# szemenyeim/DynEnv

Hardware: AMD Instinct MI355X
Metric: agent-steps/s (higher is better)
Workload: dtype f64

## Files before the change

dynenv_amd/csrc/driving_kernels.hip:

```cpp
#include "driving_dev.h"

__constant__ DrvConst C;

#include "driving_host.h"

struct DrvMailbox {
  double p1x[DRV_NS][2], p1y[DRV_NS][2], p2x[DRV_NS][2], p2y[DRV_NS][2], nx[DRV_NS], ny[DRV_NS];
  int hash[DRV_NS][2], count[DRV_NS], flag[DRV_NS];
};
struct DrvObsStage {
  float carRow[DRV_MAXA][8];
  float goal[DRV_MAXA][2];
  float shared[DRV_MAXO * 4 + DRV_MAXP * 2 + DRV_LANE_ROWS * 5];
};
#ifdef DRV_PROFILE
#define DRV_PROF(...) __VA_ARGS__
#else
#define DRV_PROF(...)
#endif
#define DRV_CLIST 128
struct __align__(16) DrvLds {
  double px[DRV_NB], py[DRV_NB], vx[DRV_NB], vy[DRV_NB], ang[DRV_NB], w[DRV_NB], vbx[DRV_NB], vby[DRV_NB], wb[DRV_NB];
  double minv[DRV_NB], iinv[DRV_NB];
  double rc[16], rs[16], rotAng[16];
// ... 684 lines not shown
  }
  double* const fX = biasLane ? L.vbx : L.vx;
  double* const fY = biasLane ? L.vby : L.vy;
  double* const fW = biasLane ? L.wb : L.w;
  const bool aDyn = bodyA < DRV_SLOT_OBST, bDyn = bodyB < DRV_SLOT_OBST;
  a.v = b.v = v2(0.0, 0.0); a.w = b.w = 0.0;
  const int nSteps = maxLevel + 1 + period * 9;
  int due = myLevel, passes = 0;
  const int ra = body_rd(bodyA), rb = body_rd(bodyB), wa = body_wr(bodyA), wb_ = body_wr(bodyB);
#define DRV_SPLIT_PASS(q)                                                                   \
  {                                                                                         \
    const V2 vr = relative_velocity(a, b, r1[q], r2[q]);                                    \
    const double vn = vdot_f(vr, n);                                                        \
    const double t0 = cq[q] + (biasLane ? -vn : vn);                                        \
    const double old = acc[q];                                                              \
    acc[q] = dms_acc_clamp0(biasLane ? t0 : -t0, nM[q], old);                               \
    const double dj = acc[q] - old;                                                         \
    const V2 jr = vrotate_f(n, v2(dj, 0.0));                                                \
    const V2 jl = vmul(n, dj);                                                              \
    const V2 jj = biasLane ? jl : jr;                                                       \
    apply_impulse(a, vneg(jj), r1[q]);                                                      \
    apply_impulse(b, jj, r2[q]);                                                            \
  }
  for (int t = 0; t < nSteps; ++t) {
    if (active && t == due && passes < 10) {
      a.v = v2(fX[ra], fY[ra]); a.w = fW[ra];
      b.v = v2(fX[rb], fY[rb]); b.w = fW[rb];
      DRV_SPLIT_PASS(0)
      if (count > 1) DRV_SPLIT_PASS(1)
      fX[wa] = a.v.x; fY[wa] = a.v.y; fW[wa] = a.w;
      fX[wb_] = b.v.x; fY[wb_] = b.v.y; fW[wb_] = b.w;
      due += period; ++passes;
    }
    __syncthreads();
  }
#undef DRV_SPLIT_PASS
  DrvSplitRet r;
  r.jt0 = jt0; r.jt1 = jt1; r.pk = pk; r.pair = pair; r.bits = bits3;
  r.jn0 = acc[0]; r.jn1 = acc[1];
  r.jb0 = lane_read_d(acc[0], (lane + 32) & 63); r.jb1 = lane_read_d(acc[1], (lane + 32) & 63);
  return r;
}

DRV_PROF(__device__ unsigned long long g_dbgw[4096 * 12];)
DRV_PROF(__device__ unsigned long long g_dbgp[4096 * 8];)
DRV_PROF(__device__ unsigned long long g_dbgr[16];)
DRV_PROF(__device__ unsigned long long g_dbgl[4096 * 8];)
DRV_PROF(__device__ unsigned long long g_dbgs[4096 * 8];)
DRV_PROF(DE_DEV int prof_any(int v) { const uint64_t m = wave_ballot(v != 0); return m ? bcast_i(v, __builtin_ctzll(m)) : 0; })
#ifndef DRV_CONTACT_INLINE
#define DRV_CONTACT_INLINE __forceinline__
#endif

DE_OOL int drv_prestep_solve(int lane, int nCarPed, int pk, int a_pair, int bodyA, int bodyB, int myLevel,
                                             int maxLevel_, int anyActive_, double jn0, double jn1, double jt0, double jt1) {
  DrvLds& L = g_L;
  DrvMailbox& M = L.u.mb;
  int a_state = pk & 0xFF;
  int a_count = (pk >> 8) & 0xFF, a_age = (pk >> 16) & 0xFF;
  bool touched = (pk >> 24) & 1, freeMe = (pk >> 25) & 1, hashSame = (pk >> 26) & 1, prevInert = (pk >> 27) & 1;
  bool skipped = (pk >> 28) & 1, slotOcc = (pk >> 29) & 1, active = (pk >> 30) & 1;
  const bool isCar = lane < (uniform_i(nCarPed) & 0xFF), isPed = lane >= DRV_SLOT_PED && lane < DRV_SLOT_PED + (uniform_i(nCarPed) >> 8);
  const int maxLevel = (int)(signed char)(uniform_i(maxLevel_) & 0xFF), period = uniform_i(maxLevel_) >> 8;
  const uint64_t activeMask = uniform_i(anyActive_) ? 1ull : 0ull;
DRV_PROF(const unsigned long long P0 = __builtin_amdgcn_s_memtime();)
  double jn[2] = {jn0, jn1}, jt[2] = {jt0, jt1};
  V2 n = v2(0.0, 0.0), r1[2], r2[2];
  r1[0] = r1[1] = r2[0] = r2[1] = v2(0.0, 0.0);
  double nMass[2] = {0.0, 0.0}, tMass[2] = {0.0, 0.0}, bias[2] = {0.0, 0.0}, bounce[2] = {0.0, 0.0}, jBias[2] = {0.0, 0.0};
  const double arb_e = 0.05 * 0.05, arb_u = 0.0 * 0.0;
  bool restIn = false;
  if (active) {
    BodyV a, b;
    body_load(L, bodyA, a);
    body_load(L, bodyB, b);
    restIn = a.v.x == 0.0 && a.v.y == 0.0 && a.w == 0.0 && b.v.x == 0.0 && b.v.y == 0.0 && b.w == 0.0;
    r1[0] = vsub(v2(M.p1x[lane][0], M.p1y[lane][0]), a.p);
    r2[0] = vsub(v2(M.p2x[lane][0], M.p2y[lane][0]), b.p);
    if (a_count > 1) {
      r1[1] = vsub(v2(M.p1x[lane][1], M.p1y[lane][1]), a.p);
      r2[1] = vsub(v2(M.p2x[lane][1], M.p2y[lane][1]), b.p);
    }
    n = v2(M.nx[lane], M.ny[lane]);
    V2 body_delta = vsub(b.p, a.p);
#pragma unroll
    for (int c = 0; c < 2; ++c) {
      if (c == 0 || a_count > 1) {
        nMass[c] = 1.0 / (k_scalar_body(a, r1[c], n) + k_scalar_body(b, r2[c], n));
        double dist = vdot_f(vadd(vsub(r2[c], r1[c]), body_delta), n);
        bias[c] = -DE_CONTACT_BIAS_COEF * fmin_cp(0.0, dist + DE_COLLISION_SLOP) / DE_DT;
        jBias[c] = 0.0;
        bounce[c] = vdot_f(relative_velocity(a, b, r1[c], r2[c]), n) * arb_e;
      }
    }
  }
  __syncthreads();
DRV_PROF(const unsigned long long P1 = __builtin_amdgcn_s_memtime();)

  velocity_update(L, lane, isCar, isPed);
DRV_PROF(int profMode = 0; const unsigned long long P2 = __builtin_amdgcn_s_memtime();)
  bool tookSplit = false;
  if (activeMask && maxLevel == 0) {
    __syncthreads();
    if (active) {
      BodyV a, b;
      body_load(L, bodyA, a);
      body_load(L, bodyB, b);
      if (a_state != ARB_FIRST) arb_warm_start(a, b, n, r1, r2, jn, jt, a_count);
      if (wave_ballot(!arb_is_bias_only(a, b, jn, jt, bounce, a_count)) == 0ull) {
DRV_PROF(profMode = 1;)
#pragma unroll 1
        for (int iter = 0; iter < 10; ++iter)
          if (wave_ballot(arb_apply_bias_only(a, b, n, r1, r2, nMass, bias, jBias, a_count)) == 0ull) break;
      } else {
DRV_PROF(profMode = 2;)
#pragma unroll 1
        for (int iter = 0; iter < 10; ++iter) arb_apply_impulse(a, b, n, r1, r2, nMass, tMass, bias, bounce, jBias, jn, jt, a_count, arb_u);
      }
      body_store_vel(L, bodyA, a);
      body_store_vel(L, bodyB, b);
    }
    __syncthreads();
  } else if (activeMask) {
    __syncthreads();
    for (int lv = 0; lv <= maxLevel; ++lv) {
      if (active && myLevel == lv && a_state != ARB_FIRST) {
        BodyV a, b;
        body_load(L, bodyA, a);
        body_load(L, bodyB, b);
        arb_warm_start(a, b, n, r1, r2, jn, jt, a_count);
        body_store_vel(L, bodyA, a);
        body_store_vel(L, bodyB, b);
      }
      __syncthreads();
    }
    BodyV a, b;
    bool biasOnly = true;
    if (active) {
      body_load(L, bodyA, a); body_load(L, bodyB, b);
      biasOnly = arb_is_bias_only(a, b, jn, jt, bounce, a_count);
    }
    const int nSteps = maxLevel + 1 + period * 9;
    int due = myLevel, passes = 0;
DRV_PROF(profMode = wave_ballot(!biasOnly) == 0ull ? 3 : 4;)
    if (wave_ballot(!biasOnly) == 0ull) {
      const int ra = body_rd(bodyA), rb = body_rd(bodyB), wa = body_wr(bodyA), wb_ = body_wr(bodyB);
      for (int t = 0; t < nSteps; ++t) {
        if (active && t == due && passes < 10) {
          a.vb = v2(L.vbx[ra], L.vby[ra]); a.wb = L.wb[ra];
          b.vb = v2(L.vbx[rb], L.vby[rb]); b.wb = L.wb[rb];
          arb_apply_bias_only(a, b, n, r1, r2, nMass, bias, jBias, a_count);
          L.vbx[wa] = a.vb.x; L.vby[wa] = a.vb.y; L.wb[wa] = a.wb;
          L.vbx[wb_] = b.vb.x; L.vby[wb_] = b.vb.y; L.wb[wb_] = b.wb;
          due += period; ++passes;
        }
        __syncthreads();
      }
    } else [[unlikely]] {
      const int bits3 = (restIn ? 1 : 0) | (bias[0] == 0.0 ? 2 : 0) | (bias[1] == 0.0 ? 4 : 0);
      const DrvSplitRet sr = drv_solve_general_split(lane, myLevel, bodyA | (bodyB << 8), maxLevel_, nMass[0], nMass[1], bias[0], bias[1], bounce[0],
                                                     bounce[1], jn[0], jn[1], jt[0], jt[1], pk, a_pair, bits3);
      lane = fresh_lane();
      pk = sr.pk; a_pair = sr.pair;
      a_state = pk & 0xFF; a_count = (pk >> 8) & 0xFF; a_age = (pk >> 16) & 0xFF;
      touched = (pk >> 24) & 1; freeMe = (pk >> 25) & 1; hashSame = (pk >> 26) & 1; prevInert = (pk >> 27) & 1;
      skipped = (pk >> 28) & 1; slotOcc = (pk >> 29) & 1; active = (pk >> 30) & 1;
      restIn = (sr.bits & 1) != 0;
      bias[0] = (sr.bits & 2) ? 0.0 : 1.0; bias[1] = (sr.bits & 4) ? 0.0 : 1.0;
      jn[0] = sr.jn0; jn[1] = sr.jn1; jBias[0] = sr.jb0; jBias[1] = sr.jb1; jt[0] = sr.jt0; jt[1] = sr.jt1;
      tookSplit = true;
    }
  }
DRV_PROF(const unsigned long long P3 = __builtin_amdgcn_s_memtime();)
  const bool wasNormal = a_state == ARB_NORMAL;
  if (active && a_state == ARB_FIRST) a_state = ARB_NORMAL;
  bool steady = true;
  if (slotOcc && !skipped) {
    steady = touched && !freeMe && hashSame;
    if (steady && a_state != ARB_IGNORE) {
      steady = a_state == ARB_NORMAL && wasNormal && restIn && L.s_jn0[lane] == jn[0] && L.s_jt0[lane] == jt[0] &&
               L.s_jn1[lane] == jn[1] && L.s_jt1[lane] == jt[1];
      if (steady) {
        const int i = a_pair >> 8, j = a_pair & 0xFF;
        steady = L.vx[i] == 0.0 && L.vy[i] == 0.0 && L.w[i] == 0.0;
        if (j < DRV_SLOT_OBST) steady = steady && L.vx[j] == 0.0 && L.vy[j] == 0.0 && L.w[j] == 0.0;
      }
    }
  }
  const bool allSteady = wave_ballot(!steady) == 0ull;
  bool inert = true;
  if (slotOcc && skipped) inert = prevInert;
  else if (slotOcc) {
    inert = touched && !freeMe &&
            (a_state == ARB_IGNORE ||
             (a_state == ARB_NORMAL && wasNormal && bias[0] == 0.0 && bias[1] == 0.0 && jn[0] == 0.0 && jt[0] == 0.0 &&
              jn[1] == 0.0 && jt[1] == 0.0 && jBias[0] == 0.0 && jBias[1] == 0.0));
  }
  if (slotOcc) {
    if (freeMe) L.s_pair[lane] = 0xFFFF;
    L.s_meta[lane] = a_state | (a_count << 8) | (a_age << 16) | (steady ? (1 << 24) : 0) | (inert ? (1 << 25) : 0);
    if (touched) { L.s_jn0[lane] = jn[0]; L.s_jt0[lane] = jt[0]; L.s_jn1[lane] = jn[1]; L.s_jt1[lane] = jt[1]; }
  }
  const bool allInert = wave_ballot(!inert) == 0ull;
DRV_PROF(if (lane == 0 && blockIdx.x < 4096) { unsigned long long* d = g_dbgp + blockIdx.x * 8; const unsigned long long P4 = __builtin_amdgcn_s_memtime(); d[2] += (P1 - P0) + ((P4 - P3) << 32); d[3] += (P2 - P1) + ((P3 - P2) << 32); })
  return (allInert ? 2 : 0) | (allSteady ? 4 : 0) | (tookSplit ? 8 : 0) DRV_PROF(| (prof_any(profMode) << 4));
}
struct ContactRet {
  uint64_t occ;
  int err;
};

__device__ DRV_CONTACT_INLINE ContactRet drv_contact_path(int lane, int cand, int dirty, int light, int A, int nCarPed, uint64_t occ) {
  const bool isCar = lane < A, isPed = lane >= DRV_SLOT_PED && lane < DRV_SLOT_PED + (nCarPed >> 8);
  DrvLds& L = g_L;
  int err = 0;
  asm volatile("" : "+v"(lane));
DRV_PROF(const unsigned long long T0 = __builtin_amdgcn_s_memtime();)
  DrvMailbox& M = L.u.mb;
  if (lane < DRV_NS) M.flag[lane] = 0;
  __syncthreads();
  bool lightOk = false;
  int savedN = uniform_i(L.clistN);
  int spair = lane < DRV_NS ? L.s_pair[lane] : -1;
DRV_PROF(int profCand = 0;)
#pragma unroll 1
  for (int mode = light ? 0 : 1; mode < 2; ++mode) {
  const int bits = mode == 0 ? dirty : cand;
  bool lightBad = false;
  int nCand = 0;
  if (mode == 1 && savedN >= 0) nCand = savedN;
  else {
#pragma unroll
  for (int i = 0; i < DRV_MAXA; ++i) {
    const bool c = (bits >> i) & 1;
    const uint64_t m = wave_ballot(c);
    if (c) {
      const int idx = nCand + (int)__builtin_amdgcn_mbcnt_hi((uint32_t)(m >> 32), __builtin_amdgcn_mbcnt_lo((uint32_t)m, 0u));
      if (idx < DRV_CLIST) L.clist[idx] = (unsigned short)((i << 8) | lane); else err |= 1;
    }
    nCand += __popcll(m);
  }
  savedN = mode == 1 && nCand <= DRV_CLIST ? nCand : -1;
  if (lane == 0) L.clistN = savedN;
  if (nCand > DRV_CLIST) nCand = DRV_CLIST;
  }
DRV_PROF(profCand += nCand;)
  __syncthreads();
DRV_PROF(const unsigned long long N1 = __builtin_amdgcn_s_memtime(); unsigned long long nMath = 0ull;)
  if (mode == 0) {
    bool owns = false;
    for (int k = lane; k < nCand; k += 64) {
      const int pr = (int)L.clist[k];
      for (uint64_t mm = occ; mm; mm &= mm - 1) owns = owns || bcast_i(spair, __builtin_ctzll(mm)) == pr;
    }
    if (wave_ballot(owns) != 0ull) continue;
  }
#pragma unroll 1
  for (int pass = 0; pass * 16 < nCand; ++pass) {
// ... 181 lines not shown
    }
    cleanSlot = cleanSlot && (myBodies & dirtyBodies) == 0;
  }
  const bool skipped = cleanSlot;
  {
    int keep = 0;
    const uint64_t skipLanes = wave_ballot(skipped);
    for (uint64_t mm = skipLanes; mm; mm &= mm - 1) keep |= bcast_i(myBodies, __builtin_ctzll(mm));
    if ((isCar || isPed) && !((keep >> lane) & 1)) { L.vbx[lane] = 0.0; L.vby[lane] = 0.0; L.wb[lane] = 0.0; }
  }

DRV_PROF(const unsigned long long U4 = __builtin_amdgcn_s_memtime();)
  const bool active = solvable && !skipped;
  const uint64_t activeMask = wave_ballot(active);
  int myLevel = 0, maxLevel = -1, period = 1;
  const int nActive = __popcll(activeMask);
  const bool lvHit = uniform_u64(c_active) == activeMask;
  if (!lvHit && lane == 0) L.sActive = activeMask;
  if (nActive == 1) maxLevel = 0;
  else if (nActive > 1 && lvHit) {
    myLevel = c_level;
    maxLevel = (int)(signed char)(uniform_i(c_meta) & 0xFF);
    period = uniform_i(c_meta) >> 8;
  } else if (nActive > 1) {
    if (!haveRank && nTouched > 1)
      for (uint64_t mm = touchedMask; mm; mm &= mm - 1) {
        int b = __builtin_ctzll(mm);
        int pk = bcast_i(a_pair, b);
        rank += (pk < a_pair) ? 1 : 0;
      }
    int bl = 0;
    const int bodyAB = bodyA | (bodyB << 8);
    for (int k = 0; k < nTouched; ++k) {
      uint64_t who = wave_ballot(active && rank == k);
      if (who == 0ull) continue;
      int b = __builtin_ctzll(who);
      const int ab = bcast_i(bodyAB, b), ba = ab & 0xFF, bb2 = ab >> 8;
      const int pa = ba < DRV_SLOT_OBST ? bcast_i(bl, ba) : 0, pb = bb2 < DRV_SLOT_OBST ? bcast_i(bl, bb2) : 0;
      const int la = pa & 0xFF, lb = pb & 0xFF;
      int lv = la > lb ? la : lb;
      const int fa = (pa >> 8) - 1, fb = (pb >> 8) - 1;
      const int lo = fa < 0 ? fb : (fb < 0 ? fa : (fa < fb ? fa : fb));
      if (lo >= 0 && lv - lo + 1 > period) period = lv - lo + 1;
      if (lane == b) myLevel = lv;
      if (lane == ba || lane == bb2) bl = (lv + 1) | (((bl >> 8) ? (bl >> 8) : lv + 1) << 8);
      maxLevel = lv > maxLevel ? lv : maxLevel;
    }
    if (lane < DRV_NS) L.sLevel[lane] = (unsigned char)myLevel;
    if (lane == 0) L.sLvMeta = (maxLevel & 0xFF) | (period << 8);
  }

DRV_PROF(const unsigned long long T2 = __builtin_amdgcn_s_memtime();)
DRV_PROF(if (lane == 0 && blockIdx.x < 4096) { unsigned long long* d = g_dbgs + blockIdx.x * 8; d[0] += U1 - T1; d[1] += U2 - U1; d[2] += U3 - U2; d[3] += U4 - U3; d[4] += T2 - U4; })
  const int solveBits = drv_prestep_solve(lane, nCarPed,
                                          (a_state & 0xFF) | ((a_count & 0xFF) << 8) | ((a_age & 0xFF) << 16) | (touched ? 1 << 24 : 0) | (freeMe ? 1 << 25 : 0) |
                                              (hashSame ? 1 << 26 : 0) | (prevInert ? 1 << 27 : 0) | (skipped ? 1 << 28 : 0) | (slotOcc ? 1 << 29 : 0) | (active ? 1 << 30 : 0),
                                          a_pair, bodyA, bodyB, myLevel, (maxLevel & 0xFF) | (period << 8), activeMask != 0ull ? 1 : 0, jn[0], jn[1], jt[0], jt[1]);
  occ &= ~freeMask;
DRV_PROF(const unsigned long long T3 = T2, T4 = T2, T5 = __builtin_amdgcn_s_memtime(); const int profModeW = (uniform_i(solveBits) >> 4) & 7;)
DRV_PROF(if (lane == 0 && blockIdx.x < 4096) { unsigned long long* d = g_dbgp + blockIdx.x * 8; d[0] += T1 - T0; d[1] += T2 - T1; d[2] += T3 - T2; d[3] += T4 - T3; d[4] += T5 - T4; d[5] += 1ull + (light ? (1ull << 16) : 0ull); d[6] += (unsigned long long)(maxLevel + 1) + ((unsigned long long)(maxLevel + 1) << (12 * profModeW)); d[7] += (unsigned long long)nTouched + ((unsigned long long)profCand << 16); })
  {
    ContactRet ret;
    ret.occ = occ; ret.err = err | (uniform_i(solveBits) & 6) | ((uniform_i(solveBits) & 8) << 1);
    return ret;
  }
}

DE_OOL int drv_partial_obs_fused(PvIn in, uint64_t seed, int A, int* envi, int env_id_offset, int e, int nPedObst, int elapsed,
                                 uint32_t episode, int noiseTypeAgents, double magn, float* __restrict__ obs, int budgetCycles);
#ifndef DRV_DEFER_MIN_CONTACT
#define DRV_DEFER_MIN_CONTACT 5
#endif
#ifndef DRV_PV_DEADLINE_PCT
#define DRV_PV_DEADLINE_PCT 110
#endif
#ifndef DRV_FUSED_AGENTS
#define DRV_FUSED_AGENTS 10
#endif
struct DrvLightRet {
  int cand, dirty, bits;
};
struct DrvSeedOnly { uint64_t seed; };
DE_OOL DrvLightRet drv_light_substep(int it_, int lane, int A_, int nPed_, int nObst_, int elapsed_,
                                                      uint32_t seedLo, uint32_t seedHi, uint32_t genv_, uint32_t episode_, int stateBits) {
  DrvLds& L = g_L;
DRV_PROF(const unsigned long long Q0 = __builtin_amdgcn_s_memtime();)
  const int lastCand = L.lastCand[lane];
  const int it = uniform_i(it_), A = uniform_i(A_), nPed = uniform_i(nPed_), nObst = uniform_i(nObst_), elapsed = uniform_i(elapsed_);
  const uint32_t genv = (uint32_t)uniform_i((int)genv_), episode = (uint32_t)uniform_i((int)episode_);
  DrvSeedOnly S;
  S.seed = ((uint64_t)(uint32_t)uniform_i((int)seedHi) << 32) | (uint64_t)(uint32_t)uniform_i((int)seedLo);
  const bool isCar = lane < A;
  const bool isPed = lane >= DRV_SLOT_PED && lane < DRV_SLOT_PED + nPed;
  const bool isBody = isCar || isPed;
  const bool vbValid = (uniform_i(stateBits) & 1) != 0;
  bool aabbValid = (uniform_i(stateBits) & 2) != 0;
    bool turned = false;
    const int bi = lane & (DRV_NB - 1), ci = lane & 15;
    int f = L.flags[bi];
    double px = L.px[bi], py = L.py[bi], vx = L.vx[bi], vy = L.vy[bi], ang = L.ang[bi];
    const double w = L.w[bi];
    const double vbx = vbValid ? L.vbx[bi] : 0.0, vby = vbValid ? L.vby[bi] : 0.0, wb = vbValid ? L.wb[bi] : 0.0;
    double rcv = L.rc[ci], rsv = L.rs[ci], rotAngv = L.rotAng[ci], cosRel0v = L.cosRel0[ci];
    const double goalx = L.goalx[ci], goaly = L.goaly[ci], dprev = L.dprev[ci], chx = L.chx[ci], chy = L.chy[ci];
    double rew = L.rewAcc[ci], posrew = L.posAcc[ci];
    int moving = L.moving[bi];
    if (!isBody) { f = 0; px = 0.0; py = 0.0; vx = 0.0; vy = 0.0; }
    if (isCar) {
      if (it == 0) {
        const int actPk = (int)L.act[lane];
// ... 271 lines not shown
    const int k = atomicAdd(&S.iso[nxt], 1);
    if (k < DRV_ISO_LIST) S.iso[DRV_ISO_HDR + nxt * DRV_ISO_LIST + k] = e;
  }
  __atomic_store_n(&S.iso_done[e], tick, __ATOMIC_RELAXED);
}

template <bool PARTIAL>
DE_DEV void drv_step_body(const DrvState& S, const int* __restrict__ actions, float* __restrict__ obs, double* __restrict__ rewards,
                          uint8_t* __restrict__ dones, float* __restrict__ pobs, int pvNoise, double pvMagn) {
  const unsigned long long isoT0 = __builtin_amdgcn_s_memtime();
DRV_PROF(const unsigned long long KS = isoT0;)
  DrvLds& L = g_L;
  int lane = threadIdx.x;
  const int tick = drv_launch_tick(S);
  if (!S.tick_src && blockIdx.x == 0 && lane == 0) { S.iso[13] = S.tick; S.iso[14] = S.pv_par; }
  const int e = drv_iso_assign(S, lane, tick);
  if (e < 0) return;
DRV_PROF(if (lane < 8 && e < 4096) { g_dbgp[e * 8 + lane] = 0ull; g_dbgs[e * 8 + lane] = 0ull; })
  const int A = S.A;
  int* envi = S.envi + (size_t)e * EI_COUNT;
  int elapsed = uniform_i(envi[EI_ELAPSED]);
  int allFinished = uniform_i(envi[EI_ALLFIN]);
  const int nPed = uniform_i(envi[EI_NPED]);
  const int nObst = uniform_i(envi[EI_NOBST]);
  const uint32_t episode = (uint32_t)uniform_i(envi[EI_EPISODE]);
  uint64_t occ = (uint64_t)(uint32_t)uniform_i(envi[EI_OCC]);
  if (occ != 0ull) __builtin_amdgcn_s_setprio(3);
  else if (PARTIAL) __builtin_amdgcn_s_setprio(1);
  const uint32_t genv = (uint32_t)(S.env_id_offset + e);

  const bool isCar = lane < A;
  const bool isPed = lane >= DRV_SLOT_PED && lane < DRV_SLOT_PED + nPed;
  const bool isBody = isCar || isPed;
  const int g_act0 = actions[((size_t)e * A + (isCar ? lane : 0)) * 2 + 0], g_act1 = actions[((size_t)e * A + (isCar ? lane : 0)) * 2 + 1];
  const int g_lastCand = S.lastcand[(size_t)e * 64 + lane];
  load_env(S, L, e, lane, A, nPed, nObst, occ);

  {
    int act0 = isCar ? g_act0 : 1, act1 = isCar ? g_act1 : 1;
    const bool bad = (unsigned)act0 > 2u || (unsigned)act1 > 2u;
    if (bad) { act0 = 1; act1 = 1; }
    if (lane < 16) L.act[lane] = (unsigned char)(act0 | (act1 << 2));
    const bool anyBad = wave_ballot(bad) != 0ull;
    if (lane == 0) L.stepErr = anyBad ? 2 : 0;
  }
  int finishedAt = -1;
  if (lane < 16) { L.rewAcc[lane] = 0.0; L.posAcc[lane] = 0.0; }
  bool aabbValid = false;
  L.lastCand[lane] = g_lastCand;
  if (lane == 0) { L.clistN = -1; L.sActive = ~0ull; L.sLvMeta = 0; }
  bool inertAll = (uniform_i(envi[EI_PAD]) & 1) != 0;
  bool steadyAll = (uniform_i(envi[EI_PAD]) & 2) != 0;
  bool vbValid = (uniform_i(envi[EI_PAD]) & 4) != 0;
  int nFast = 0, nQuiet = 0, nContact = 0, nSlots = 0, nWhyCand = 0, nWhyMoving = 0, nWhyInert = 0, nSteady = 0, nLight = 0, nSplit = 0;
  __syncthreads();

DRV_PROF(const unsigned long long K0 = __builtin_amdgcn_s_memtime(); unsigned long long tPh1 = 0, tBroad = 0, tFast = 0, tCont = 0, tBook = 0;)
  bool lightOff = false;
  for (int it = 0; it < 10; ++it) {
    lane = fresh_lane();
DRV_PROF(const unsigned long long A0 = __builtin_amdgcn_s_memtime();)
    const DrvLightRet lr = drv_light_substep(it, lane, A, nPed, nObst, elapsed, (uint32_t)S.seed, (uint32_t)(S.seed >> 32), genv, episode,
                                             (vbValid ? 1 : 0) | (aabbValid ? 2 : 0));
    const int cand = lr.cand, dirty = lr.dirty;
    const bool candMoving = (lr.bits & 1) != 0, removed = (lr.bits & 2) != 0;
    aabbValid = true;
DRV_PROF(const unsigned long long A1 = A0;)
    const uint64_t anyCand = wave_ballot(cand != 0);
    const bool candChanged = wave_ballot((lr.bits & 4) != 0) != 0ull, anyMoving = wave_ballot(candMoving) != 0ull;
    if (candChanged && lane == 0) L.clistN = -1;
    const bool quiescent = inertAll && !candChanged && !anyMoving;
    const bool steadyOk = !quiescent && steadyAll && wave_ballot(removed) == 0ull;
    const bool anyDirty = wave_ballot(dirty != 0) != 0ull;
    bool replay = steadyOk && !anyDirty;
    const bool light = steadyOk && anyDirty && !lightOff;
    if (!(anyCand == 0ull && occ == 0ull) && !quiescent && !replay) { if (candChanged) nWhyCand++; else if (anyMoving) nWhyMoving++; else nWhyInert++; }

DRV_PROF(const unsigned long long A2 = __builtin_amdgcn_s_memtime(); bool tookContact = false;)
    if (anyCand == 0ull && occ == 0ull) nFast++; else if (quiescent) nQuiet++; else if (replay) nSteady++; else nContact++;
    nSlots += __popcll(occ);
    if ((anyCand == 0ull && occ == 0ull) || quiescent) {
      velocity_update_ool(A | (nPed << 8));
      if (anyCand == 0ull && occ == 0ull) steadyAll = false;
      vbValid = false;
    } else if (!replay) {
DRV_PROF(tookContact = true;)
      __builtin_amdgcn_s_setprio(3);
      ContactRet cr = drv_contact_path(lane, cand, dirty, light ? 1 : 0, A, A | (nPed << 8), occ);
      lane = fresh_lane();
      if (wave_ballot((cr.err & 1) != 0) != 0ull && lane == 0) L.stepErr |= 1;
      if (light && !(uniform_i(cr.err >> 3) & 1)) lightOff = true;
      if (uniform_i(cr.err >> 3) & 1) {
        replay = true; nLight++;
      } else {
        nSplit += uniform_i(cr.err >> 4) & 1;
        occ = uniform_u64(cr.occ);
        inertAll = (uniform_i(cr.err >> 1) & 1) != 0;
        steadyAll = (uniform_i(cr.err >> 2) & 1) != 0;
        vbValid = true;
      }
    }
    if (replay) {
      velocity_update_ool(A | (nPed << 8));
      vbValid = true;
    }
    __syncthreads();

DRV_PROF(const unsigned long long A3 = __builtin_amdgcn_s_memtime(); tPh1 += A1 - A0; tBroad += A2 - A1; if (tookContact) tCont += A3 - A2; else tFast += A3 - A2;)
    elapsed += 1;
    bool notDone = false;
    if (isCar) { int f = L.flags[lane]; notDone = !(CF_FIN(f) && !CF_CRASHED(f)); }
    const bool allFin = wave_ballot(notDone) == 0ull;
    if (!allFinished && allFin) {
      allFinished = 1;
      finishedAt = elapsed;
    }
  }
  lane = fresh_lane();
  const double teamReward = finishedAt >= 0 ? 0.0 + (double)(DRV_MAX_TIME - finishedAt) / 100.0 : 0.0;

DRV_PROF(const unsigned long long K1 = __builtin_amdgcn_s_memtime();)
  double* er = S.epr + (size_t)e * 16 + (isCar ? lane : 0);
  double* ep = S.epr + (size_t)S.E * 16 + (size_t)e * 16 + (isCar ? lane : 0);
  const double g_er = *er, g_ep = *ep;
  const int cl = lane < 10 ? lane : 0;
  const int g_cnt = envi[EI_N_FAST + cl];
  const int g_err = envi[EI_ERR];
  double rew = 0.0, posrew = 0.0;
  if (isCar) {
    rew = L.rewAcc[lane] + teamReward;
    posrew = L.posAcc[lane] + dm_max(0.0, teamReward);
    rewards[(size_t)e * A + lane] = rew;
  }
  if (lane == 0) {
    dones[e] = (uint8_t)(elapsed >= DRV_MAX_TIME);
    envi[EI_ELAPSED] = elapsed; envi[EI_ALLFIN] = allFinished; envi[EI_OCC] = (int)(uint32_t)occ;
    envi[EI_PAD] = (inertAll ? 1 : 0) | (steadyAll ? 2 : 0) | (vbValid ? 4 : 0);
  }
  const int errBits = uniform_i(L.stepErr);
  S.lastcand[(size_t)e * 64 + lane] = L.lastCand[lane];
  store_env(S, L, e, lane, A, nPed, occ);
  if (obs) write_full_obs_ool(lane, A, nPed, nObst, S.obs_dim, obs + (size_t)e * A * S.obs_dim);
  if (isCar) { *er = g_er + rew; *ep = g_ep + posrew; }
  {
    static_assert(EI_N_QUIET == EI_N_FAST + 1 && EI_N_CONTACT == EI_N_FAST + 2 && EI_N_SLOTS == EI_N_FAST + 3 && EI_N_WHY_CAND == EI_N_FAST + 4 &&
                  EI_N_WHY_MOVING == EI_N_FAST + 5 && EI_N_WHY_INERT == EI_N_FAST + 6 && EI_N_STEADY == EI_N_FAST + 7 && EI_N_LIGHT == EI_N_FAST + 8 && EI_N_SPLIT == EI_N_FAST + 9,
                  "the diagnostic counters are consecutive");
    const int add = lane == 0 ? nFast : lane == 1 ? nQuiet : lane == 2 ? nContact : lane == 3 ? nSlots : lane == 4 ? nWhyCand : lane == 5 ? nWhyMoving :
                    lane == 6 ? nWhyInert : lane == 7 ? nSteady : lane == 8 ? nLight : nSplit;
    if (lane < 10) envi[EI_N_FAST + lane] = g_cnt + add;
  }
  if (errBits && lane == 0) envi[EI_ERR] = g_err | errBits;
  int fusedAgents = !(PARTIAL && pobs) ? 0 : nContact >= DRV_DEFER_MIN_CONTACT ? 0 : (A < DRV_FUSED_AGENTS ? A : DRV_FUSED_AGENTS);
  int budget = 0;
  if (PARTIAL && pobs && S.iso_on >= 2) {
    const int slowest = uniform_i(S.iso[3 + tick % 3]);
    if (slowest > 0) {
      budget = (slowest / 100) * DRV_PV_DEADLINE_PCT - (int)(__builtin_amdgcn_s_memtime() - isoT0);
      fusedAgents = budget > 0 ? A : 0;
    }
  }
  drv_iso_report(S, e, fresh_lane(), isoT0, tick);
  if (PARTIAL && fusedAgents > 0) {
    __builtin_amdgcn_s_setprio(0);
    PvIn in;
    in.px = in.py = in.ang = in.ox = in.oy = in.gx = in.gy = 0.0; in.flags = 0;
    if (lane < DRV_NB && (lane < A || (lane >= DRV_SLOT_PED && lane < DRV_SLOT_PED + nPed))) {
      in.px = L.px[lane]; in.py = L.py[lane]; in.ang = L.ang[lane]; in.flags = L.flags[lane];
    }
    if (lane < nObst) { in.ox = L.ox[lane]; in.oy = L.oy[lane]; }
    if (lane < A) { in.gx = L.goalx[lane]; in.gy = L.goaly[lane]; }
    fusedAgents = drv_partial_obs_fused(in, S.seed, S.A, S.envi, S.env_id_offset, e, nPed | (nObst << 8), elapsed, episode, pvNoise | (fusedAgents << 8), pvMagn,
                                        pobs, budget);
  }
  if (PARTIAL && fresh_lane() == 0) {
    envi[EI_DEFER_OBS] = fusedAgents;
    if (pobs && fusedAgents < A) {
      const int pv = drv_launch_pv(S);
      const int k = atomicAdd(&S.pvq[16 * pv], 1);
      if (k < S.E) S.pvq[32 + pv * S.E + k] = e;
      else envi[EI_ERR] = envi[EI_ERR] | 4;
    }
  }
DRV_PROF(if (lane == 0 && e < 4096) { unsigned long long* d = g_dbgw + e * 12; const unsigned long long KE = __builtin_amdgcn_s_memtime(); d[0] = KE - KS; d[1] = nContact; d[2] = __popcll(occ); d[3] = nSteady + nQuiet; d[4] = K0 - KS; d[5] = tPh1; d[6] = tBroad; d[7] = tFast; d[8] = tCont; d[9] = (K1 - K0) - tPh1 - tBroad - tFast - tCont; d[10] = KE - K1; d[11] = ((unsigned long long)__builtin_amdgcn_s_getreg(63508) << 32) | (unsigned long long)__builtin_amdgcn_s_getreg(63492); })
}

extern "C" __global__ void drv_tick_advance_kernel(DrvState S, int flipPv) {
  if (threadIdx.x == 0 && blockIdx.x == 0) { S.iso[13] = (S.iso[13] + 1) % (3 * (1 << 28)); if (flipPv) S.iso[14] = S.iso[14] ^ 1; }
}

extern "C" __global__ void __launch_bounds__(64, DRV_WAVES_PER_SIMD)
drv_step_kernel(DrvState S, const int* __restrict__ actions, float* __restrict__ obs, double* __restrict__ rewards,
                uint8_t* __restrict__ dones) {
  drv_step_body<false>(S, actions, obs, rewards, dones, nullptr, 0, 0.0);
}
extern "C" __global__ void __launch_bounds__(64, DRV_WAVES_PER_SIMD)
drv_step_partial_kernel(DrvState S, const int* __restrict__ actions, double* __restrict__ rewards, uint8_t* __restrict__ dones,
                        float* __restrict__ pobs, int pvNoise, double pvMagn) {
  drv_step_body<true>(S, actions, nullptr, rewards, dones, pobs, pvNoise, pvMagn);
}

extern "C" __global__ void __launch_bounds__(64) drv_obs_kernel(DrvState S, float* __restrict__ obs) {
  DrvLds& L = g_L;
  const int e = blockIdx.x, lane = threadIdx.x, A = S.A;
  const int* envi = S.envi + (size_t)e * EI_COUNT;
  const int nPed = uniform_i(envi[EI_NPED]), nObst = uniform_i(envi[EI_NOBST]);
  load_env(S, L, e, lane, A, nPed, nObst, 0ull);
  write_full_obs_ool(lane, A, nPed, nObst, S.obs_dim, obs + (size_t)e * A * S.obs_dim);
}

DE_DEV void road_get_spot(const DrvRoad& r, int lane, int spot, V2& pos, double& angle) {
  int end = lane >= r.nLanes ? 1 : 0;
  V2 p = end ? r.p1 : r.p0;
  V2 spotDir = vmul(end ? vneg(r.dir) : r.dir, r.followDist);
  V2 laneDir = vmul(end ? r.normal : vneg(r.normal), r.width);
  double l = (double)(end ? lane - r.nLanes : lane) + 0.5;
  pos = vadd(vadd(p, vmul(laneDir, l)), vmul(spotDir, (double)spot));
  angle = dm_atan2(spotDir.y, spotDir.x);
}
DE_DEV V2 road_get_walk_spot(const DrvRoad& r, int side, double length, double width) {
  V2 w0 = r.walk[side][0], w1 = r.walk[side][1];
  V2 center = vadd(w0, vmul(vsub(w1, w0), length));
  double f = width * r.width;
  V2 off = vmul(vmul(r.normal, f), side ? 1.0 : -1.0);
  return vadd(center, off);
}

extern "C" __global__ void __launch_bounds__(64) drv_reset_kernel(DrvState S) {
  const int e = blockIdx.x * blockDim.x + threadIdx.x;
  if (e >= S.E) return;
  const size_t E = (size_t)S.E;
  const int A = S.A;
  int* envi = S.envi + (size_t)e * EI_COUNT;
  const uint32_t ep = (uint32_t)envi[EI_EPISODE];
  const uint32_t genv = (uint32_t)(S.env_id_offset + e);
  for (int k = 0; k < DRV_NB; ++k) {
    for (int f = 0; f < BF_COUNT; ++f) S.body[(size_t)f * E * DRV_NB + (size_t)e * DRV_NB + k] = 0.0;
    S.flags[(size_t)e * DRV_NB + k] = 0;
// ... 218 lines not shown
```

Before: 260.9 million.

## Split prestep solver into single/multi-level variants and hoist split solve to caller

Splits the out-of-line prestep solver into a single-level entry and a templated multi-level entry. The rarely used general split solve moves out of the solver into the caller, with its inputs returned packed in a 12-double vector, and the slot-verdict bookkeeping is factored into a shared helper. The ten per-step diagnostic counters are packed into two 4-bit-field integers. The goal is to cut register pressure and code size on the hot path so the common single-level case is lighter. The cost is extra argument marshalling when the split path runs, and the 4-bit counters can overflow if a counter exceeds 15 within one call.

```diff
diff --git a/dynenv_amd/csrc/driving_kernels.hip b/dynenv_amd/csrc/driving_kernels.hip
--- a/dynenv_amd/csrc/driving_kernels.hip
+++ b/dynenv_amd/csrc/driving_kernels.hip
@@ -760,14 +760,55 @@
 #define DRV_CONTACT_INLINE __forceinline__
 #endif
 
-DE_OOL int drv_prestep_solve(int lane, int nCarPed, int pk, int a_pair, int bodyA, int bodyB, int myLevel,
-                                             int maxLevel_, int anyActive_, double jn0, double jn1, double jt0, double jt1) {
+DE_DEV int drv_slot_verdicts(int lane, int pk, int a_pair, bool restIn, bool biasZ0, bool biasZ1, double jn0, double jn1, double jt0, double jt1,
+                             double jBias0, double jBias1, bool tookSplit) {
+  DrvLds& L = g_L;
+  int a_state = pk & 0xFF;
+  const int a_count = (pk >> 8) & 0xFF, a_age = (pk >> 16) & 0xFF;
+  const bool touched = (pk >> 24) & 1, freeMe = (pk >> 25) & 1, hashSame = (pk >> 26) & 1, prevInert = (pk >> 27) & 1;
+  const bool skipped = (pk >> 28) & 1, slotOcc = (pk >> 29) & 1, active = (pk >> 30) & 1;
+  const bool wasNormal = a_state == ARB_NORMAL;
+  if (active && a_state == ARB_FIRST) a_state = ARB_NORMAL;
+  bool steady = true;
+  if (slotOcc && !skipped) {
+    steady = touched && !freeMe && hashSame;
+    if (steady && a_state != ARB_IGNORE) {
+      steady = a_state == ARB_NORMAL && wasNormal && restIn && L.s_jn0[lane] == jn0 && L.s_jt0[lane] == jt0 &&
+               L.s_jn1[lane] == jn1 && L.s_jt1[lane] == jt1;
+      if (steady) {
+        const int i = a_pair >> 8, j = a_pair & 0xFF;
+        steady = L.vx[i] == 0.0 && L.vy[i] == 0.0 && L.w[i] == 0.0;
+        if (j < DRV_SLOT_OBST) steady = steady && L.vx[j] == 0.0 && L.vy[j] == 0.0 && L.w[j] == 0.0;
+      }
+    }
+  }
+  const bool allSteady = wave_ballot(!steady) == 0ull;
+  bool inert = true;
+  if (slotOcc && skipped) inert = prevInert;
+  else if (slotOcc) {
+    inert = touched && !freeMe &&
+            (a_state == ARB_IGNORE ||
+             (a_state == ARB_NORMAL && wasNormal && biasZ0 && biasZ1 && jn0 == 0.0 && jt0 == 0.0 &&
+              jn1 == 0.0 && jt1 == 0.0 && jBias0 == 0.0 && jBias1 == 0.0));
+  }
+  if (slotOcc) {
+    if (freeMe) L.s_pair[lane] = 0xFFFF;
+    L.s_meta[lane] = a_state | (a_count << 8) | (a_age << 16) | (steady ? (1 << 24) : 0) | (inert ? (1 << 25) : 0);
+    if (touched) { L.s_jn0[lane] = jn0; L.s_jt0[lane] = jt0; L.s_jn1[lane] = jn1; L.s_jt1[lane] = jt1; }
+  }
+  const bool allInert = wave_ballot(!inert) == 0ull;
+  return (allInert ? 2 : 0) | (allSteady ? 4 : 0) | (tookSplit ? 8 : 0);
+}
+typedef double DrvSolveRet __attribute__((ext_vector_type(12)));
+DE_DEV double drv_pack2(int lo, int hi) { return __hiloint2double(hi, lo); }
+template <bool MULTI>
+DE_DEV DrvSolveRet drv_prestep_solve_body(int lane, int nCarPed, int pk, int a_pair, int bodyA, int bodyB, int myLevel,
+                                          int maxLevel_, int anyActive_, double jn0, double jn1, double jt0, double jt1) {
   DrvLds& L = g_L;
   DrvMailbox& M = L.u.mb;
-  int a_state = pk & 0xFF;
-  int a_count = (pk >> 8) & 0xFF, a_age = (pk >> 16) & 0xFF;
-  bool touched = (pk >> 24) & 1, freeMe = (pk >> 25) & 1, hashSame = (pk >> 26) & 1, prevInert = (pk >> 27) & 1;
-  bool skipped = (pk >> 28) & 1, slotOcc = (pk >> 29) & 1, active = (pk >> 30) & 1;
+  const int a_state = pk & 0xFF;
+  const int a_count = (pk >> 8) & 0xFF;
+  const bool active = (pk >> 30) & 1;
   const bool isCar = lane < (uniform_i(nCarPed) & 0xFF), isPed = lane >= DRV_SLOT_PED && lane < DRV_SLOT_PED + (uniform_i(nCarPed) >> 8);
   const int maxLevel = (int)(signed char)(uniform_i(maxLevel_) & 0xFF), period = uniform_i(maxLevel_) >> 8;
   const uint64_t activeMask = uniform_i(anyActive_) ? 1ull : 0ull;
@@ -807,8 +848,7 @@
 
   velocity_update(L, lane, isCar, isPed);
 DRV_PROF(int profMode = 0; const unsigned long long P2 = __builtin_amdgcn_s_memtime();)
-  bool tookSplit = false;
-  if (activeMask && maxLevel == 0) {
+  if (!MULTI && activeMask) {
     __syncthreads();
     if (active) {
       BodyV a, b;
@@ -829,7 +869,7 @@
       body_store_vel(L, bodyB, b);
     }
     __syncthreads();
-  } else if (activeMask) {
+  } else if (MULTI) {
     __syncthreads();
     for (int lv = 0; lv <= maxLevel; ++lv) {
       if (active && myLevel == lv && a_state != ARB_FIRST) {
@@ -865,53 +905,33 @@
         __syncthreads();
       }
     } else [[unlikely]] {
+DRV_PROF(if (lane == 0 && blockIdx.x < 4096) { unsigned long long* d = g_dbgp + blockIdx.x * 8; const unsigned long long P3 = __builtin_amdgcn_s_memtime(); d[2] += P1 - P0; d[3] += (P2 - P1) + ((P3 - P2) << 32); })
       const int bits3 = (restIn ? 1 : 0) | (bias[0] == 0.0 ? 2 : 0) | (bias[1] == 0.0 ? 4 : 0);
-      const DrvSplitRet sr = drv_solve_general_split(lane, myLevel, bodyA | (bodyB << 8), maxLevel_, nMass[0], nMass[1], bias[0], bias[1], bounce[0],
-                                                     bounce[1], jn[0], jn[1], jt[0], jt[1], pk, a_pair, bits3);
-      lane = fresh_lane();
-      pk = sr.pk; a_pair = sr.pair;
-      a_state = pk & 0xFF; a_count = (pk >> 8) & 0xFF; a_age = (pk >> 16) & 0xFF;
-      touched = (pk >> 24) & 1; freeMe = (pk >> 25) & 1; hashSame = (pk >> 26) & 1; prevInert = (pk >> 27) & 1;
-      skipped = (pk >> 28) & 1; slotOcc = (pk >> 29) & 1; active = (pk >> 30) & 1;
-      restIn = (sr.bits & 1) != 0;
-      bias[0] = (sr.bits & 2) ? 0.0 : 1.0; bias[1] = (sr.bits & 4) ? 0.0 : 1.0;
-      jn[0] = sr.jn0; jn[1] = sr.jn1; jBias[0] = sr.jb0; jBias[1] = sr.jb1; jt[0] = sr.jt0; jt[1] = sr.jt1;
-      tookSplit = true;
+      DrvSolveRet r;
+      r[0] = nMass[0]; r[1] = nMass[1]; r[2] = bias[0]; r[3] = bias[1]; r[4] = bounce[0]; r[5] = bounce[1];
+      r[6] = jn[0]; r[7] = jn[1]; r[8] = jt[0]; r[9] = jt[1];
+      r[10] = drv_pack2(pk, a_pair);
+      r[11] = drv_pack2(1 | (bits3 << 8) | (myLevel << 16), bodyA | (bodyB << 8) | (maxLevel_ << 16));
+      return r;
     }
   }
 DRV_PROF(const unsigned long long P3 = __builtin_amdgcn_s_memtime();)
-  const bool wasNormal = a_state == ARB_NORMAL;
-  if (active && a_state == ARB_FIRST) a_state = ARB_NORMAL;
-  bool steady = true;
-  if (slotOcc && !skipped) {
-    steady = touched && !freeMe && hashSame;
-    if (steady && a_state != ARB_IGNORE) {
-      steady = a_state == ARB_NORMAL && wasNormal && restIn && L.s_jn0[lane] == jn[0] && L.s_jt0[lane] == jt[0] &&
-               L.s_jn1[lane] == jn[1] && L.s_jt1[lane] == jt[1];
-      if (steady) {
-        const int i = a_pair >> 8, j = a_pair & 0xFF;
-        steady = L.vx[i] == 0.0 && L.vy[i] == 0.0 && L.w[i] == 0.0;
-        if (j < DRV_SLOT_OBST) steady = steady && L.vx[j] == 0.0 && L.vy[j] == 0.0 && L.w[j] == 0.0;
-      }
-    }
-  }
-  const bool allSteady = wave_ballot(!steady) == 0ull;
-  bool inert = true;
-  if (slotOcc && skipped) inert = prevInert;
-  else if (slotOcc) {
-    inert = touched && !freeMe &&
-            (a_state == ARB_IGNORE ||
-             (a_state == ARB_NORMAL && wasNormal && bias[0] == 0.0 && bias[1] == 0.0 && jn[0] == 0.0 && jt[0] == 0.0 &&
-              jn[1] == 0.0 && jt[1] == 0.0 && jBias[0] == 0.0 && jBias[1] == 0.0));
-  }
-  if (slotOcc) {
-    if (freeMe) L.s_pair[lane] = 0xFFFF;
-    L.s_meta[lane] = a_state | (a_count << 8) | (a_age << 16) | (steady ? (1 << 24) : 0) | (inert ? (1 << 25) : 0);
-    if (touched) { L.s_jn0[lane] = jn[0]; L.s_jt0[lane] = jt[0]; L.s_jn1[lane] = jn[1]; L.s_jt1[lane] = jt[1]; }
-  }
-  const bool allInert = wave_ballot(!inert) == 0ull;
+  const int bits = drv_slot_verdicts(lane, pk, a_pair, restIn, bias[0] == 0.0, bias[1] == 0.0, jn[0], jn[1], jt[0], jt[1], jBias[0], jBias[1], false);
 DRV_PROF(if (lane == 0 && blockIdx.x < 4096) { unsigned long long* d = g_dbgp + blockIdx.x * 8; const unsigned long long P4 = __builtin_amdgcn_s_memtime(); d[2] += (P1 - P0) + ((P4 - P3) << 32); d[3] += (P2 - P1) + ((P3 - P2) << 32); })
-  return (allInert ? 2 : 0) | (allSteady ? 4 : 0) | (tookSplit ? 8 : 0) DRV_PROF(| (prof_any(profMode) << 4));
+  DrvSolveRet r;
+  r[11] = drv_pack2(bits DRV_PROF(| (prof_any(profMode) << 4)), 0);
+  return r;
+}
+DE_OOL int drv_prestep_solve(int lane, int nCarPed, int pk, int a_pair, int bodyA, int bodyB, int anyActive_, double jn0, double jn1, double jt0,
+                             double jt1) {
+  return __double2loint(drv_prestep_solve_body<false>(lane, nCarPed, pk, a_pair, bodyA, bodyB, 0, 1 << 8 , anyActive_, jn0, jn1, jt0, jt1)[11]);
+}
+DE_OOL DrvSolveRet drv_prestep_solve_multi(int lane, int nCarPed, int pk, int a_pair, int bodyA, int bodyB, int myLevel, int maxLevel_, double jn0,
+                                           double jn1, double jt0, double jt1) {
+  return drv_prestep_solve_body<true>(lane, nCarPed, pk, a_pair, bodyA, bodyB, myLevel, maxLevel_, 1, jn0, jn1, jt0, jt1);
+}
+DE_OOL int drv_split_verdicts(int lane, int pk, int a_pair, int bits3, double jn0, double jn1, double jBias0, double jBias1, double jt0, double jt1) {
+  return drv_slot_verdicts(lane, pk, a_pair, (bits3 & 1) != 0, (bits3 & 2) != 0, (bits3 & 4) != 0, jn0, jn1, jt0, jt1, jBias0, jBias1, true);
 }
 struct ContactRet {
   uint64_t occ;
@@ -1199,10 +1219,24 @@
 
 DRV_PROF(const unsigned long long T2 = __builtin_amdgcn_s_memtime();)
 DRV_PROF(if (lane == 0 && blockIdx.x < 4096) { unsigned long long* d = g_dbgs + blockIdx.x * 8; d[0] += U1 - T1; d[1] += U2 - U1; d[2] += U3 - U2; d[3] += U4 - U3; d[4] += T2 - U4; })
-  const int solveBits = drv_prestep_solve(lane, nCarPed,
-                                          (a_state & 0xFF) | ((a_count & 0xFF) << 8) | ((a_age & 0xFF) << 16) | (touched ? 1 << 24 : 0) | (freeMe ? 1 << 25 : 0) |
-                                              (hashSame ? 1 << 26 : 0) | (prevInert ? 1 << 27 : 0) | (skipped ? 1 << 28 : 0) | (slotOcc ? 1 << 29 : 0) | (active ? 1 << 30 : 0),
-                                          a_pair, bodyA, bodyB, myLevel, (maxLevel & 0xFF) | (period << 8), activeMask != 0ull ? 1 : 0, jn[0], jn[1], jt[0], jt[1]);
+  const int pkArg = (a_state & 0xFF) | ((a_count & 0xFF) << 8) | ((a_age & 0xFF) << 16) | (touched ? 1 << 24 : 0) | (freeMe ? 1 << 25 : 0) |
+                    (hashSame ? 1 << 26 : 0) | (prevInert ? 1 << 27 : 0) | (skipped ? 1 << 28 : 0) | (slotOcc ? 1 << 29 : 0) | (active ? 1 << 30 : 0);
+  int solveBits;
+  if (activeMask == 0ull || maxLevel == 0) {
+    solveBits = drv_prestep_solve(lane, nCarPed, pkArg, a_pair, bodyA, bodyB, activeMask != 0ull ? 1 : 0, jn[0], jn[1], jt[0], jt[1]);
+  } else {
+    const DrvSolveRet sv = drv_prestep_solve_multi(lane, nCarPed, pkArg, a_pair, bodyA, bodyB, myLevel, (maxLevel & 0xFF) | (period << 8), jn[0], jn[1], jt[0], jt[1]);
+    solveBits = __double2loint(sv[11]);
+    if (uniform_i(solveBits) & 1) [[unlikely]] {
+      const int w1 = __double2hiint(sv[11]);
+DRV_PROF(const unsigned long long S0 = __builtin_amdgcn_s_memtime();)
+      const DrvSplitRet sr = drv_solve_general_split(fresh_lane(), (solveBits >> 16) & 0xFF, w1 & 0xFFFF, w1 >> 16, sv[0], sv[1], sv[2], sv[3], sv[4], sv[5],
+                                                     sv[6], sv[7], sv[8], sv[9], __double2loint(sv[10]), __double2hiint(sv[10]), (solveBits >> 8) & 7);
+DRV_PROF(const unsigned long long S1 = __builtin_amdgcn_s_memtime();)
+      solveBits = drv_split_verdicts(fresh_lane(), sr.pk, sr.pair, sr.bits, sr.jn0, sr.jn1, sr.jb0, sr.jb1, sr.jt0, sr.jt1) DRV_PROF(| (4 << 4));
+DRV_PROF(if (fresh_lane() == 0 && blockIdx.x < 4096) { unsigned long long* d = g_dbgp + blockIdx.x * 8; d[3] += (S1 - S0) << 32; d[2] += (__builtin_amdgcn_s_memtime() - S1) << 32; })
+    }
+  }
   occ &= ~freeMask;
 DRV_PROF(const unsigned long long T3 = T2, T4 = T2, T5 = __builtin_amdgcn_s_memtime(); const int profModeW = (uniform_i(solveBits) >> 4) & 7;)
 DRV_PROF(if (lane == 0 && blockIdx.x < 4096) { unsigned long long* d = g_dbgp + blockIdx.x * 8; d[0] += T1 - T0; d[1] += T2 - T1; d[2] += T3 - T2; d[3] += T4 - T3; d[4] += T5 - T4; d[5] += 1ull + (light ? (1ull << 16) : 0ull); d[6] += (unsigned long long)(maxLevel + 1) + ((unsigned long long)(maxLevel + 1) << (12 * profModeW)); d[7] += (unsigned long long)nTouched + ((unsigned long long)profCand << 16); })
@@ -1580,7 +1614,10 @@
   bool inertAll = (uniform_i(envi[EI_PAD]) & 1) != 0;
   bool steadyAll = (uniform_i(envi[EI_PAD]) & 2) != 0;
   bool vbValid = (uniform_i(envi[EI_PAD]) & 4) != 0;
-  int nFast = 0, nQuiet = 0, nContact = 0, nSlots = 0, nWhyCand = 0, nWhyMoving = 0, nWhyInert = 0, nSteady = 0, nLight = 0, nSplit = 0;
+  unsigned cntA = 0u, cntB = 0u;
+#define DRV_CNT(ei) (1u << (4 * ((ei) - EI_N_FAST)))
+#define DRV_CNT_GET(ei) ((int)((cntA >> (4 * ((ei) - EI_N_FAST))) & 15u))
+  static_assert(EI_N_STEADY - EI_N_FAST == 7 && EI_N_SLOTS - EI_N_FAST == 3 && DRV_NS * 10 < 256, "seven counters of four bits in cntA, the slot sum in eight bits of cntB");
   __syncthreads();
 
 DRV_PROF(const unsigned long long K0 = __builtin_amdgcn_s_memtime(); unsigned long long tPh1 = 0, tBroad = 0, tFast = 0, tCont = 0, tBook = 0;)
@@ -1602,11 +1639,11 @@
     const bool anyDirty = wave_ballot(dirty != 0) != 0ull;
     bool replay = steadyOk && !anyDirty;
     const bool light = steadyOk && anyDirty && !lightOff;
-    if (!(anyCand == 0ull && occ == 0ull) && !quiescent && !replay) { if (candChanged) nWhyCand++; else if (anyMoving) nWhyMoving++; else nWhyInert++; }
+    if (!(anyCand == 0ull && occ == 0ull) && !quiescent && !replay) cntA += candChanged ? DRV_CNT(EI_N_WHY_CAND) : anyMoving ? DRV_CNT(EI_N_WHY_MOVING) : DRV_CNT(EI_N_WHY_INERT);
 
 DRV_PROF(const unsigned long long A2 = __builtin_amdgcn_s_memtime(); bool tookContact = false;)
-    if (anyCand == 0ull && occ == 0ull) nFast++; else if (quiescent) nQuiet++; else if (replay) nSteady++; else nContact++;
-    nSlots += __popcll(occ);
+    cntA += (anyCand == 0ull && occ == 0ull) ? DRV_CNT(EI_N_FAST) : quiescent ? DRV_CNT(EI_N_QUIET) : replay ? DRV_CNT(EI_N_STEADY) : DRV_CNT(EI_N_CONTACT);
+    cntB += (unsigned)__popcll(occ);
     if ((anyCand == 0ull && occ == 0ull) || quiescent) {
       velocity_update_ool(A | (nPed << 8));
       if (anyCand == 0ull && occ == 0ull) steadyAll = false;
@@ -1619,9 +1656,9 @@
       if (wave_ballot((cr.err & 1) != 0) != 0ull && lane == 0) L.stepErr |= 1;
       if (light && !(uniform_i(cr.err >> 3) & 1)) lightOff = true;
       if (uniform_i(cr.err >> 3) & 1) {
-        replay = true; nLight++;
+        replay = true; cntB = (unsigned)uniform_i((int)(cntB + (1u << 8)));
       } else {
-        nSplit += uniform_i(cr.err >> 4) & 1;
+        cntB = (unsigned)uniform_i((int)(cntB + ((unsigned)(uniform_i(cr.err >> 4) & 1) << 12)));
         occ = uniform_u64(cr.occ);
         inertAll = (uniform_i(cr.err >> 1) & 1) != 0;
         steadyAll = (uniform_i(cr.err >> 2) & 1) != 0;
@@ -1633,6 +1670,7 @@
       vbValid = true;
     }
     __syncthreads();
+    if (!PARTIAL) lane = fresh_lane();
 
 DRV_PROF(const unsigned long long A3 = __builtin_amdgcn_s_memtime(); tPh1 += A1 - A0; tBroad += A2 - A1; if (tookContact) tCont += A3 - A2; else tFast += A3 - A2;)
     elapsed += 1;
@@ -1674,12 +1712,11 @@
     static_assert(EI_N_QUIET == EI_N_FAST + 1 && EI_N_CONTACT == EI_N_FAST + 2 && EI_N_SLOTS == EI_N_FAST + 3 && EI_N_WHY_CAND == EI_N_FAST + 4 &&
                   EI_N_WHY_MOVING == EI_N_FAST + 5 && EI_N_WHY_INERT == EI_N_FAST + 6 && EI_N_STEADY == EI_N_FAST + 7 && EI_N_LIGHT == EI_N_FAST + 8 && EI_N_SPLIT == EI_N_FAST + 9,
                   "the diagnostic counters are consecutive");
-    const int add = lane == 0 ? nFast : lane == 1 ? nQuiet : lane == 2 ? nContact : lane == 3 ? nSlots : lane == 4 ? nWhyCand : lane == 5 ? nWhyMoving :
-                    lane == 6 ? nWhyInert : lane == 7 ? nSteady : lane == 8 ? nLight : nSplit;
+    const int add = (int)(cl == 3 ? (cntB & 0xFFu) : cl < 8 ? (cntA >> (4 * cl)) & 15u : (cntB >> (4 * cl - 24)) & 15u);
     if (lane < 10) envi[EI_N_FAST + lane] = g_cnt + add;
   }
   if (errBits && lane == 0) envi[EI_ERR] = g_err | errBits;
-  int fusedAgents = !(PARTIAL && pobs) ? 0 : nContact >= DRV_DEFER_MIN_CONTACT ? 0 : (A < DRV_FUSED_AGENTS ? A : DRV_FUSED_AGENTS);
+  int fusedAgents = !(PARTIAL && pobs) ? 0 : DRV_CNT_GET(EI_N_CONTACT) >= DRV_DEFER_MIN_CONTACT ? 0 : (A < DRV_FUSED_AGENTS ? A : DRV_FUSED_AGENTS);
   int budget = 0;
   if (PARTIAL && pobs && S.iso_on >= 2) {
     const int slowest = uniform_i(S.iso[3 + tick % 3]);
@@ -1710,8 +1747,11 @@
       else envi[EI_ERR] = envi[EI_ERR] | 4;
     }
   }
-DRV_PROF(if (lane == 0 && e < 4096) { unsigned long long* d = g_dbgw + e * 12; const unsigned long long KE = __builtin_amdgcn_s_memtime(); d[0] = KE - KS; d[1] = nContact; d[2] = __popcll(occ); d[3] = nSteady + nQuiet; d[4] = K0 - KS; d[5] = tPh1; d[6] = tBroad; d[7] = tFast; d[8] = tCont; d[9] = (K1 - K0) - tPh1 - tBroad - tFast - tCont; d[10] = KE - K1; d[11] = ((unsigned long long)__builtin_amdgcn_s_getreg(63508) << 32) | (unsigned long long)__builtin_amdgcn_s_getreg(63492); })
-}
+DRV_PROF(if (lane == 0 && e < 4096) { unsigned long long* d = g_dbgw + e * 12; const unsigned long long KE = __builtin_amdgcn_s_memtime(); d[0] = KE - KS; d[1] = DRV_CNT_GET(EI_N_CONTACT); d[2] = __popcll(occ); d[3] = DRV_CNT_GET(EI_N_STEADY) + DRV_CNT_GET(EI_N_QUIET); d[4] = K0 - KS; d[5] = tPh1; d[6] = tBroad; d[7] = tFast; d[8] = tCont; d[9] = (K1 - K0) - tPh1 - tBroad - tFast - tCont; d[10] = KE - K1; d[11] = ((unsigned long long)__builtin_amdgcn_s_getreg(63508) << 32) | (unsigned long long)__builtin_amdgcn_s_getreg(63492); })
+}
+
+#undef DRV_CNT
+#undef DRV_CNT_GET
 
 extern "C" __global__ void drv_tick_advance_kernel(DrvState S, int flipPv) {
   if (threadIdx.x == 0 && blockIdx.x == 0) { S.iso[13] = (S.iso[13] + 1) % (3 * (1 << 28)); if (flipPv) S.iso[14] = S.iso[14] ^ 1; }
```

Result: faster. 264.5 million, median of 6 (+1.4%).
